# StanfordASL/RiskAverseTrajOpt

Measured on AMD Instinct MI355X. Metric: SAA constraint-eval throughput, higher is better.
Workload: dtype f32

## Files before the change

riskaversetrajopt_amd/csrc/rato_sample_launch.h:

```cpp
#pragma once
#include "rato_common.h"
#include "rato_rows_plan.h"
#include "rato_select.h"

namespace rato {

struct StatsRequest {
  void* workspace;
  double* out;
  double alpha;
  float thr;
  int flags;
  bool ok(const float* Z) const { return !workspace || (Z && out && alpha > 0.0 && alpha <= 1.0); }
};
template <class Params>
StatsRequest stats_request(const Params* p) {
  return {p->stats_workspace, p->stats_out, p->stats_alpha, p->stats_thr, p->stats_flags};
}

struct StatsPlacement {
  rato_sel::StatsTail tail;
  int grid;
  size_t lds;
  bool behind;
};
template <int NT>
int place_stats(const StatsRequest& rq, int64_t M, int grid, size_t lds, bool may_carry, StatsPlacement& sp) {
  sp = {{}, grid, lds, rq.workspace && !may_carry};
  if (!rq.workspace || !may_carry) return RATO_OK;
  const int extra = rato_sel::stats_tail_workgroups<NT>(M, sp.tail.G);
  if (extra < 0) return RATO_EINVAL;
  sp.tail.ws = static_cast<rato_sel::Workspace*>(rq.workspace);
  sp.tail.out = rq.out;
  sp.tail.alpha = rq.alpha;
  sp.tail.thr = rq.thr;
  sp.tail.n_prod = grid;
  rato_sel::stats_rank(M, rq.alpha, sp.tail.k, sp.tail.var_is_max);
  sp.grid = grid + extra;
  if (sp.lds < rato_sel::rs_body_lds_bytes<NT>()) sp.lds = rato_sel::rs_body_lds_bytes<NT>();
  return RATO_OK;
}
inline int stats_behind(const StatsRequest& rq, bool behind, const float* Z, int64_t M, void* stream) {
  if (!behind) return RATO_OK;
  return rato_risk_stats(Z, M, rq.alpha, rq.thr, rq.workspace, rato_risk_stats_workspace_bytes(M), rq.out, stream);
}

struct RowsLaunch {
  rato_rows_plan plan;
  unsigned* queue;
  StatsPlacement stats;
};
template <int NT, class PlanWith>
int prepare_rows_launch(PlanWith&& plan_with, TileQueuePool& pool, unsigned* (*resolve)(), hipStream_t st,
                        const StatsRequest& rq, int64_t M, size_t lds, RowsLaunch& rl) {
  rl.plan = plan_with(true);
  rl.queue = rl.plan.wants_queue ? pool.take(st, resolve) : nullptr;
  if (rl.plan.wants_queue && !rl.queue) rl.plan = plan_with(false);
  return place_stats<NT>(rq, M, rl.plan.workgroups, lds, !rl.queue, rl.stats);
}

}
```

riskaversetrajopt_amd/csrc/rato_select.h:

```cpp
#ifndef RATO_SELECT_H
#define RATO_SELECT_H

#include <math.h>

#include "rato_common.h"

namespace rato_sel {

constexpr unsigned long long RS_COOP_WAIT_TICKS = 10ull * 100000000ull;
constexpr int B1 = 2048, B2 = 2048, B3 = 1024;
constexpr int RS_MAX_BLOCKS = 1024;

struct Workspace {
  unsigned hist1[B1];
  unsigned hist2[B2];
  unsigned hist3[B3];
  double blockpart[RS_MAX_BLOCKS][6];
  float tstar;
  unsigned nblocks;
  unsigned magic;
  unsigned ticket;
  unsigned sig[8];
};
constexpr int SIG_Z_COUNT = 0, SIG_Z_READY = 2;
constexpr unsigned RS_MAGIC = 0x52A70517u;

__device__ __forceinline__ unsigned key_of(float f) {
  unsigned u = __float_as_uint(f);
  if (u == 0x80000000u) u = 0u;
  return (u & 0x80000000u) ? ~u : (u | 0x80000000u);
}
__device__ __forceinline__ float value_of(unsigned k) {
  const unsigned u = (k & 0x80000000u) ? (k & 0x7fffffffu) : ~k;
  return __uint_as_float(u);
}

template <int NB, int NT = RATO_BLOCK>
__device__ void find_bin(const unsigned* __restrict__ hist, unsigned k, unsigned& bin, unsigned& krem) {
  constexpr int PER = NB / NT;
  static_assert(PER >= 1 && PER * NT == NB, "bins must divide evenly over the threads");
  __shared__ unsigned wsum[NT / RATO_WAVE];
  __shared__ unsigned res[2];
  const int tid = threadIdx.x, lane = tid & 63, wave = tid >> 6;
  unsigned local[PER], tot = 0;
#pragma unroll
  for (int i = 0; i < PER; ++i) {
    local[i] = hist[tid * PER + i];
    tot += local[i];
  }
  const unsigned incl = rato::wave_scan_dpp(tot);
  if (lane == 63) wsum[wave] = incl;
  __syncthreads();
  unsigned base = 0;
  for (int w = 0; w < wave; ++w) base += wsum[w];
  unsigned excl = base + incl - tot;
  if (k >= excl && k < excl + tot) {
    unsigned run = excl;
#pragma unroll
    for (int i = 0; i < PER; ++i) {
      if (k >= run && k < run + local[i]) {
        res[0] = tid * PER + i;
        res[1] = k - run;
      }
      run += local[i];
    }
  }
  __syncthreads();
  bin = res[0];
  krem = res[1];
  __syncthreads();
}

template <int NB, int NT = RATO_BLOCK>
__device__ void flush_hist(unsigned* lds_hist, unsigned* __restrict__ ghist) {
  __syncthreads();
  for (int i = threadIdx.x; i < NB; i += NT) {
    const unsigned c = lds_hist[i];
    if (c) atomicAdd(&ghist[i], c);
  }
}


__device__ bool wait_signal(unsigned* flag) {
  __shared__ unsigned s_ok;
  if (threadIdx.x == 0) {
    const unsigned long long t_start = wall_clock64();
    unsigned ok = 1;
    for (unsigned tries = 0; __hip_atomic_load(flag, __ATOMIC_RELAXED, __HIP_MEMORY_SCOPE_AGENT) == 0u; ++tries) {
      if ((tries & 255u) == 255u && wall_clock64() - t_start > RS_COOP_WAIT_TICKS) {
        ok = 0;
        break;
      }
      __builtin_amdgcn_s_sleep(32);
    }
    __builtin_amdgcn_fence(__ATOMIC_ACQUIRE, "agent");
    s_ok = ok;
  }
  __syncthreads();
  const bool ok = s_ok != 0;
  __syncthreads();
  return ok;
}


constexpr long RS_SMALL_MAX = 12 * 1024;
constexpr int RS_COOP_KEYS = 16;
constexpr int RS_COOP_MAX_WG = 64;

template <int NB, int NT>
__device__ bool find_bin_coop(const unsigned* __restrict__ hist, unsigned k, unsigned expected, unsigned& bin,
                              unsigned& krem, unsigned& bincount) {
  constexpr int PER = NB / NT;
  static_assert(PER >= 1 && PER * NT == NB, "bins must divide evenly over the threads");
  __shared__ unsigned wsum[NT / RATO_WAVE];
  __shared__ unsigned res[3];
  const int tid = threadIdx.x, lane = tid & 63, wave = tid >> 6;
  const unsigned long long t_start = wall_clock64();
  for (unsigned tries = 0;; ++tries) {
    unsigned local[PER], tot = 0;
#pragma unroll
    for (int i = 0; i < PER; ++i) {
      local[i] = __hip_atomic_load(const_cast<unsigned*>(hist) + tid * PER + i, __ATOMIC_RELAXED, __HIP_MEMORY_SCOPE_AGENT);
      tot += local[i];
    }
    const unsigned incl = rato::wave_scan_dpp(tot);
    if (lane == 63) wsum[wave] = incl;
    __syncthreads();
    unsigned base = 0, grand = 0;
    for (int w = 0; w < NT / RATO_WAVE; ++w) {
      const unsigned v = wsum[w];
      if (w < wave) base += v;
      grand += v;
    }
    if (grand == expected) {
      const unsigned excl = base + incl - tot;
      if (k >= excl && k < excl + tot) {
        unsigned run = excl;
#pragma unroll
        for (int i = 0; i < PER; ++i) {
          if (k >= run && k < run + local[i]) {
            res[0] = tid * PER + i;
            res[1] = k - run;
            res[2] = local[i];
          }
          run += local[i];
        }
      }
      __syncthreads();
      bin = res[0];
      krem = res[1];
      bincount = res[2];
      __syncthreads();
      return true;
    }
    if (grand > expected) return false;
    if ((tries & 1023u) == 1023u) {
      if (tid == 0) res[0] = (wall_clock64() - t_start > RS_COOP_WAIT_TICKS) ? 1u : 0u;
      __syncthreads();
      const unsigned expired = res[0];
      __syncthreads();
      if (expired) return false;
    }
    __syncthreads();
    if (tries < 64) __builtin_amdgcn_s_sleep(4); else __builtin_amdgcn_s_sleep(32);
  }
}


__device__ __forceinline__ unsigned wave_min_u32_dpp(unsigned a) {
  const int top = (int)0xffffffffu;
  a = min(a, (unsigned)__builtin_amdgcn_update_dpp(top, (int)a, 0x111, 0xf, 0xf, false));
  a = min(a, (unsigned)__builtin_amdgcn_update_dpp(top, (int)a, 0x112, 0xf, 0xf, false));
  a = min(a, (unsigned)__builtin_amdgcn_update_dpp(top, (int)a, 0x114, 0xf, 0xf, false));
  a = min(a, (unsigned)__builtin_amdgcn_update_dpp(top, (int)a, 0x118, 0xf, 0xf, false));
  a = min(a, (unsigned)__builtin_amdgcn_update_dpp(top, (int)a, 0x142, 0xa, 0xf, false));
  a = min(a, (unsigned)__builtin_amdgcn_update_dpp(top, (int)a, 0x143, 0xc, 0xf, false));
  return (unsigned)__builtin_amdgcn_readlane((int)a, 63);
}
__device__ __forceinline__ unsigned wave_max_u32_dpp(unsigned a) {
  a = max(a, (unsigned)__builtin_amdgcn_update_dpp(0, (int)a, 0x111, 0xf, 0xf, false));
  a = max(a, (unsigned)__builtin_amdgcn_update_dpp(0, (int)a, 0x112, 0xf, 0xf, false));
  a = max(a, (unsigned)__builtin_amdgcn_update_dpp(0, (int)a, 0x114, 0xf, 0xf, false));
  a = max(a, (unsigned)__builtin_amdgcn_update_dpp(0, (int)a, 0x118, 0xf, 0xf, false));
  a = max(a, (unsigned)__builtin_amdgcn_update_dpp(0, (int)a, 0x142, 0xa, 0xf, false));
  a = max(a, (unsigned)__builtin_amdgcn_update_dpp(0, (int)a, 0x143, 0xc, 0xf, false));
  return (unsigned)__builtin_amdgcn_readlane((int)a, 63);
}

constexpr int RS_CAND_MAX = 256;

template <int NT>
__device__ void rs_small_body(const float* __restrict__ Z, long M, double alpha, unsigned k, int var_is_max, float thr,
                              double* __restrict__ out, unsigned* sig, unsigned* h, double* red, float* redmax,
                              unsigned* magic = nullptr) {
  constexpr int KEYS = (int)(RS_SMALL_MAX / NT), NW = NT / RATO_WAVE;
  static_assert(RS_CAND_MAX + 8 <= B1, "the candidate list reuses the histogram's LDS");
  if (sig) {
    const bool tagged = !magic || *magic == RS_MAGIC;
    const bool ok = tagged && wait_signal(sig + SIG_Z_READY);
    if (!ok) {
      if (threadIdx.x < RATO_N_STATS) out[threadIdx.x] = __longlong_as_double(0x7ff8000000000000LL);
      if (magic && threadIdx.x == 0) *magic = 0u;
      return;
    }
    if (threadIdx.x == 0) __hip_atomic_store(sig + SIG_Z_READY, 0u, __ATOMIC_RELAXED, __HIP_MEMORY_SCOPE_AGENT);
  }
  const int tid = threadIdx.x;
  const int n = (int)M;
#ifdef RATO_RS_DIAG
  if (tid == 0) out[16 + 0] = (double)wall_clock64();
#endif
  unsigned key[KEYS];
  double sum = 0.0, cnt = 0.0;
  float mx = -INFINITY;
  unsigned kmin = 0xffffffffu, kmax = 0u;
  {
    float z[KEYS];
#pragma unroll
    for (int u = 0; u < KEYS; ++u) {
      const int i = tid + u * NT;
      z[u] = (i < n) ? Z[i] : 0.0f;
    }
#pragma unroll
    for (int u = 0; u < KEYS; ++u) {
      const int i = tid + u * NT;
      key[u] = key_of(z[u]);
      if (i < n) {
        sum += (double)z[u];
        cnt += (z[u] <= thr) ? 1.0 : 0.0;
        mx = fmaxf(mx, z[u]);
        kmin = min(kmin, key[u]);
        kmax = max(kmax, key[u]);
      }
    }
  }
  unsigned* mm = reinterpret_cast<unsigned*>(red);
  kmin = wave_min_u32_dpp(kmin);
  kmax = wave_max_u32_dpp(kmax);
  if ((tid & 63) == 0) {
    mm[tid >> 6] = kmin;
    mm[NW + (tid >> 6)] = kmax;
  }
  __syncthreads();
#pragma unroll
  for (int w = 0; w < NW; ++w) {
    kmin = min(kmin, mm[w]);
    kmax = max(kmax, mm[NW + w]);
  }
#ifdef RATO_RS_DIAG
  if (tid == 0) out[16 + 1] = (double)wall_clock64();
#endif
  unsigned lo = kmin, krem = k;
  const unsigned range = kmax - kmin;
  int sh = (range == 0u) ? 0 : (32 - __clz((int)range)) - 11;
  if (sh < 0) sh = 0;
  unsigned width = 0u;
  unsigned tkey = 0u;
  for (int level = 0;; ++level) {
    for (int i = tid; i < B1; i += NT) h[i] = 0;
    __syncthreads();
    {
      unsigned run_bin = 0xffffffffu, run_cnt = 0;
#pragma unroll
      for (int u = 0; u < KEYS; ++u) {
        const int i = tid + u * NT;
        const unsigned rel = key[u] - lo;
        if (i < n && (level == 0 || (key[u] >= lo && rel < width))) {
          const unsigned bin = rel >> sh;
          if (bin != run_bin) {
            if (run_cnt) atomicAdd(&h[run_bin], run_cnt);
            run_bin = bin;
            run_cnt = 0;
// ... 19 lines not shown
      unsigned* cand = h;
      if (tid == 0) h[B1 - 2] = 0u;
      __syncthreads();
#pragma unroll
      for (int u = 0; u < KEYS; ++u) {
        const int i = tid + u * NT;
        if (i < n && key[u] >= lo && key[u] - lo < width) cand[atomicAdd(&h[B1 - 2], 1u)] = key[u];
      }
      __syncthreads();
      if (tid < (int)c) {
        const unsigned x = cand[tid];
        unsigned lt = 0, le = 0;
        for (unsigned j = 0; j < c; ++j) {
          const unsigned y = cand[j];
          lt += (y < x) ? 1u : 0u;
          le += (y <= x) ? 1u : 0u;
        }
        if (lt <= krem && krem < le) h[B1 - 1] = x;
      }
      __syncthreads();
      tkey = h[B1 - 1];
      break;
    }
    sh = (sh > 11) ? sh - 11 : 0;
  }
#ifdef RATO_RS_DIAG
  if (tid == 0) out[16 + 6] = (double)wall_clock64();
#endif
  const float t = value_of(tkey);
  double tail = 0.0, ngt = 0.0, neq = 0.0;
#pragma unroll
  for (int u = 0; u < KEYS; ++u) {
    const int i = tid + u * NT;
    if (i < n) {
      const float z = value_of(key[u]);
      tail += (key[u] > tkey) ? ((double)z - (double)t) : 0.0;
      ngt += (key[u] > tkey) ? 1.0 : 0.0;
      neq += (key[u] == tkey) ? 1.0 : 0.0;
    }
  }
#ifdef RATO_RS_DIAG
  if (tid == 0) out[16 + 7] = (double)wall_clock64();
#endif
  sum = rato::wave_sum_dpp(sum);
  cnt = rato::wave_sum_dpp(cnt);
  tail = rato::wave_sum_dpp(tail);
  ngt = rato::wave_sum_dpp(ngt);
  neq = rato::wave_sum_dpp(neq);
  mx = rato::wave_max_dpp(mx);
  __syncthreads();
  if ((tid & 63) == 0) {
    const int w = tid >> 6;
    red[0 * NW + w] = sum; red[1 * NW + w] = cnt; red[2 * NW + w] = tail; red[3 * NW + w] = ngt; red[4 * NW + w] = neq;
    redmax[w] = mx;
  }
  __syncthreads();
  if (tid < RATO_WAVE) {
    static_assert(NT / RATO_WAVE <= 16, "one DPP row folds the wave totals");
    const bool in = tid < NT / RATO_WAVE;
    const double S = rato::row16_sum_dpp(in ? red[0 * NW + tid] : 0.0), C = rato::row16_sum_dpp(in ? red[1 * NW + tid] : 0.0);
    const double T = rato::row16_sum_dpp(in ? red[2 * NW + tid] : 0.0), NG = rato::row16_sum_dpp(in ? red[3 * NW + tid] : 0.0);
    const double NE = rato::row16_sum_dpp(in ? red[4 * NW + tid] : 0.0);
    const double m = (double)rato::row16_max_dpp(in ? redmax[tid] : -INFINITY);
    if (tid == 15) {
      out[0] = var_is_max ? m : (double)t;
      out[1] = (double)t + (T / (double)M) / alpha;
      out[2] = C / (double)M;
      out[3] = S / (double)M;
      out[4] = m;
      out[5] = C;
      out[6] = T;
      out[7] = (double)k;
      out[8] = NG;
      out[9] = NE;
      out[10] = (double)t;
#ifdef RATO_RS_DIAG
      out[16 + 8] = (double)wall_clock64();
#endif
    }
  }
}


template <int NT>
__device__ void rs_coop_body(const float* __restrict__ Z, long M, double alpha, unsigned k, int var_is_max, float thr, int G,
                             Workspace* __restrict__ ws, double* __restrict__ out, int bid, int companion, unsigned* h,
                             double* red) {
  constexpr int NW = NT / RATO_WAVE;
  const int tid = threadIdx.x;
  if (ws->magic != RS_MAGIC) {
    if (bid == 0 && tid < RATO_N_STATS) out[tid] = __longlong_as_double(0x7ff8000000000000LL);
    return;
  }
  const bool z_ok = companion ? wait_signal(ws->sig + SIG_Z_READY) : true;
  __shared__ unsigned last_flag;
  const int n = (int)M;
  unsigned key[RS_COOP_KEYS];
  double sum = 0.0, cnt = 0.0;
  float mx = -INFINITY;
  {
    float z[RS_COOP_KEYS];
#pragma unroll
    for (int u = 0; u < RS_COOP_KEYS; ++u) {
      const int i = (u * G + bid) * NT + tid;
      z[u] = (i < n) ? Z[i] : 0.0f;
    }
    for (int i = tid; i < B1; i += NT) h[i] = 0;
    __syncthreads();
    unsigned run_bin = 0xffffffffu, run_cnt = 0;
#pragma unroll
    for (int u = 0; u < RS_COOP_KEYS; ++u) {
      const int i = (u * G + bid) * NT + tid;
      key[u] = key_of(z[u]);
      if (i < n) {
        const unsigned bin = key[u] >> 21;
        if (bin != run_bin) {
          if (run_cnt) atomicAdd(&h[run_bin], run_cnt);
          run_bin = bin;
          run_cnt = 0;
        }
        ++run_cnt;
        sum += (double)z[u];
        cnt += (z[u] <= thr) ? 1.0 : 0.0;
        mx = fmaxf(mx, z[u]);
      }
    }
    if (run_cnt) atomicAdd(&h[run_bin], run_cnt);
  }
  flush_hist<B1, NT>(h, ws->hist1);
  unsigned b1 = 0, k1 = 0, c1 = 0, b2 = 0, k2 = 0, c2 = 0, b3 = 0, k3 = 0, c3 = 0;
  bool ok = z_ok && find_bin_coop<B1, NT>(ws->hist1, k, (unsigned)n, b1, k1, c1);
  for (int i = tid; i < B2; i += NT) h[i] = 0;
  __syncthreads();
#pragma unroll
  for (int u = 0; u < RS_COOP_KEYS; ++u) {
    const int i = (u * G + bid) * NT + tid;
    if (i < n && (key[u] >> 21) == b1) atomicAdd(&h[(key[u] >> 10) & (B2 - 1)], 1u);
  }
  flush_hist<B2, NT>(h, ws->hist2);
  ok = ok && find_bin_coop<B2, NT>(ws->hist2, k1, c1, b2, k2, c2);
  for (int i = tid; i < B3; i += NT) h[i] = 0;
  __syncthreads();
  const unsigned prefix = (b1 << 11) | b2;
#pragma unroll
  for (int u = 0; u < RS_COOP_KEYS; ++u) {
    const int i = (u * G + bid) * NT + tid;
    if (i < n && (key[u] >> 10) == prefix) atomicAdd(&h[key[u] & (B3 - 1)], 1u);
  }
  flush_hist<B3, NT>(h, ws->hist3);
  ok = ok && find_bin_coop<B3, NT>(ws->hist3, k2, c2, b3, k3, c3);
  if (!ok) {
    if (tid < RATO_N_STATS) out[tid] = __longlong_as_double(0x7ff8000000000000LL);
    if (tid == 0) ws->magic = 0;
    return;
  }
  const unsigned tkey = (b1 << 21) | (b2 << 10) | b3;
  const float t = value_of(tkey);
  double tail = 0.0, ngt = 0.0, neq = 0.0;
#pragma unroll
  for (int u = 0; u < RS_COOP_KEYS; ++u) {
    const int i = (u * G + bid) * NT + tid;
    if (i < n) {
      const float z = value_of(key[u]);
      tail += (key[u] > tkey) ? ((double)z - (double)t) : 0.0;
      ngt += (key[u] > tkey) ? 1.0 : 0.0;
      neq += (key[u] == tkey) ? 1.0 : 0.0;
    }
  }
  sum = rato::wave_sum_dpp(sum);
  cnt = rato::wave_sum_dpp(cnt);
  tail = rato::wave_sum_dpp(tail);
  ngt = rato::wave_sum_dpp(ngt);
  neq = rato::wave_sum_dpp(neq);
  mx = rato::wave_max_dpp(mx);
  if ((tid & 63) == 0) {
    const int w = tid >> 6;
    red[0 * NW + w] = sum; red[1 * NW + w] = cnt; red[2 * NW + w] = (double)mx; red[3 * NW + w] = tail; red[4 * NW + w] = ngt; red[5 * NW + w] = neq;
  }
  __syncthreads();
  if (tid < RATO_WAVE) {
    const bool in = tid < NT / RATO_WAVE;
    const double S = rato::row16_sum_dpp(in ? red[0 * NW + tid] : 0.0), C = rato::row16_sum_dpp(in ? red[1 * NW + tid] : 0.0);
    const double T = rato::row16_sum_dpp(in ? red[3 * NW + tid] : 0.0), NG = rato::row16_sum_dpp(in ? red[4 * NW + tid] : 0.0);
    const double NE = rato::row16_sum_dpp(in ? red[5 * NW + tid] : 0.0);
    const double m = (double)rato::row16_max_dpp(in ? (float)red[2 * NW + tid] : -INFINITY);
    if (tid == 15) {
      double* bp = ws->blockpart[bid];
      bp[0] = S; bp[1] = C; bp[2] = m; bp[3] = T; bp[4] = NG; bp[5] = NE;
      const unsigned tk = __hip_atomic_fetch_add(&ws->ticket, 1u, __ATOMIC_ACQ_REL, __HIP_MEMORY_SCOPE_AGENT);
      last_flag = (tk == (unsigned)G - 1u);
    }
  }
  __syncthreads();
  if (!last_flag) return;
  for (int i = tid; i < B1 + B2 + B3; i += NT) ws->hist1[i] = 0;
  if (tid == 0) {
    ws->ticket = 0;
    if (companion) __hip_atomic_store(ws->sig + SIG_Z_READY, 0u, __ATOMIC_RELAXED, __HIP_MEMORY_SCOPE_AGENT);
  }
  if (tid >= RATO_WAVE) return;
  double s = 0, c = 0, m = -INFINITY, tl = 0, g = 0, e = 0;
  if (tid < G) {
    const double* bp = ws->blockpart[tid];
    s = __hip_atomic_load(bp + 0, __ATOMIC_RELAXED, __HIP_MEMORY_SCOPE_AGENT);
    c = __hip_atomic_load(bp + 1, __ATOMIC_RELAXED, __HIP_MEMORY_SCOPE_AGENT);
    m = __hip_atomic_load(bp + 2, __ATOMIC_RELAXED, __HIP_MEMORY_SCOPE_AGENT);
    tl = __hip_atomic_load(bp + 3, __ATOMIC_RELAXED, __HIP_MEMORY_SCOPE_AGENT);
    g = __hip_atomic_load(bp + 4, __ATOMIC_RELAXED, __HIP_MEMORY_SCOPE_AGENT);
    e = __hip_atomic_load(bp + 5, __ATOMIC_RELAXED, __HIP_MEMORY_SCOPE_AGENT);
  }
  s = rato::wave_sum_dpp(s);
  c = rato::wave_sum_dpp(c);
  tl = rato::wave_sum_dpp(tl);
  g = rato::wave_sum_dpp(g);
  e = rato::wave_sum_dpp(e);
  m = (double)rato::wave_max_dpp((float)m);
  if (tid != 0) return;
  out[0] = var_is_max ? m : (double)t;
  out[1] = (double)t + (tl / (double)M) / alpha;
  out[2] = c / (double)M;
  out[3] = s / (double)M;
  out[4] = m;
  out[5] = c;
  out[6] = tl;
  out[7] = (double)k;
  out[8] = g;
  out[9] = e;
  out[10] = (double)t;
}


struct StatsTail {
  Workspace* ws;
  double* out;
  double alpha;
  unsigned k;
  int var_is_max;
  float thr;
  int G;
  int n_prod;
  __device__ bool is_stats(int b) const { return ws && b >= n_prod; }
};

inline void stats_rank(int64_t M, double alpha, unsigned& k, int& var_is_max) {
  long xth = (long)floor(alpha * (double)M);
  long kk = (long)M - xth - 1;
  var_is_max = 0;
  if (kk < 0) {
    kk = 0;
    var_is_max = 1;
  }
  k = (unsigned)kk;
}

template <int NT>
inline int stats_tail_workgroups(int64_t M, int& G) {
  if (M <= RS_SMALL_MAX) {
    G = 0;
    return 1;
  }
  long g = (M + (long)NT * 4 - 1) / ((long)NT * 4);
  if (g > RS_COOP_MAX_WG) g = RS_COOP_MAX_WG;
  if ((long)g * NT * RS_COOP_KEYS < M) return -1;
  G = (int)g;
  return (int)g;
}

template <int NT>
__device__ __forceinline__ void stats_tail_run(const StatsTail& t, const float* __restrict__ Z, long M, unsigned char* lds) {
  unsigned* h = reinterpret_cast<unsigned*>(lds);
  double* red = reinterpret_cast<double*>(h + B1);
  float* redmax = reinterpret_cast<float*>(red + 6 * (NT / RATO_WAVE));
  if (t.G == 0) rs_small_body<NT>(Z, M, t.alpha, t.k, t.var_is_max, t.thr, t.out, t.ws->sig, h, red, redmax, &t.ws->magic);
  else rs_coop_body<NT>(Z, M, t.alpha, t.k, t.var_is_max, t.thr, t.G, t.ws, t.out, (int)blockIdx.x - t.n_prod, 1, h, red);
}

template <int NT>
constexpr size_t rs_body_lds_bytes() { return sizeof(unsigned) * B1 + sizeof(double) * 6 * (NT / RATO_WAVE) + sizeof(float) * (NT / RATO_WAVE); }


}
#endif
```

riskaversetrajopt_amd/csrc/stats.hip:

```cpp
#include <stdlib.h>

#include <atomic>

#include "rato_common.h"
#include "rato_select.h"

namespace {
using namespace rato_sel;

constexpr int SP_COLS = 16, SP_ROWS = 64;

template <typename T>
__device__ __forceinline__ void sum_partials_block(int col_block, const T* __restrict__ part, int nblocks,
                                                   int ncols, double scale, double* __restrict__ out) {
  __shared__ double red[SP_ROWS][SP_COLS + 1];
  const int cx = threadIdx.x % SP_COLS, ry = threadIdx.x / SP_COLS;
  const int c = col_block * SP_COLS + cx;
  double a0 = 0.0, a1 = 0.0, a2 = 0.0, a3 = 0.0;
  if (c < ncols) {
    int b = ry;
    for (; b + 3 * SP_ROWS < nblocks; b += 4 * SP_ROWS) {
      const T v0 = part[(size_t)b * ncols + c];
      const T v1 = part[(size_t)(b + SP_ROWS) * ncols + c];
      const T v2 = part[(size_t)(b + 2 * SP_ROWS) * ncols + c];
// ... 172 lines not shown
    if (blockIdx.x == 0) ws->tstar = t;
  }
}

__global__ __launch_bounds__(RATO_BLOCK) void rs_final(long M, double alpha, unsigned k, int var_is_max, int nblocks,
                                                        Workspace* __restrict__ ws, double* __restrict__ out) {
  const bool ok = ws->magic == RS_MAGIC;
  for (int i = threadIdx.x; i < B1 + B2 + B3; i += RATO_BLOCK) ws->hist1[i] = 0;
  if (!ok) {
    if (threadIdx.x < RATO_N_STATS) out[threadIdx.x] = __longlong_as_double(0x7ff8000000000000LL);
    return;
  }
  if (threadIdx.x >= RATO_WAVE) return;
  const int lane = threadIdx.x;
  double s = 0, c = 0, m = -INFINITY, tail = 0, ngt = 0, neq = 0;
  for (int b = lane; b < nblocks; b += RATO_WAVE) {
    s += ws->blockpart[b][0];
    c += ws->blockpart[b][1];
    m = fmax(m, ws->blockpart[b][2]);
    tail += ws->blockpart[b][3];
    ngt += ws->blockpart[b][4];
    neq += ws->blockpart[b][5];
  }
  s = rato::wave_sum(s);
  c = rato::wave_sum(c);
  tail = rato::wave_sum(tail);
  ngt = rato::wave_sum(ngt);
  neq = rato::wave_sum(neq);
#pragma unroll
  for (int off = 32; off > 0; off >>= 1) m = fmax(m, __shfl_xor(m, off, RATO_WAVE));
  if (lane != 0) return;
  const double t = (double)ws->tstar;
  out[0] = var_is_max ? m : t;
  out[1] = t + (tail / (double)M) / alpha;
  out[2] = c / (double)M;
  out[3] = s / (double)M;
  out[4] = m;
  out[5] = c;
  out[6] = tail;
  out[7] = (double)k;
  out[8] = ngt;
  out[9] = neq;
  out[10] = t;
}

constexpr int RS1_T = 1024;

__global__ __launch_bounds__(RS1_T) void rs_small(const float* __restrict__ Z, long M, double alpha, unsigned k,
                                                  int var_is_max, float thr, double* __restrict__ out,
                                                  const float* __restrict__ part, int nblocks, int ncols,
                                                  double scale, double* __restrict__ sums_out) {
  if (blockIdx.x > 0) {
    sum_partials_block(blockIdx.x - 1, part, nblocks, ncols, scale, sums_out);
    return;
  }
  __shared__ unsigned h[B1];
  __shared__ double red[5 * (RS1_T / RATO_WAVE)];
  __shared__ float redmax[RS1_T / RATO_WAVE];
  rs_small_body<RS1_T>(Z, M, alpha, k, var_is_max, thr, out, nullptr, h, red, redmax);
}

__global__ __launch_bounds__(RS1_T) void rs_small_tab(const rato::BatchProb* __restrict__ tab, long M) {
  __shared__ unsigned h[B1];
  __shared__ double red[5 * (RS1_T / RATO_WAVE)];
  __shared__ float redmax[RS1_T / RATO_WAVE];
  const rato::BatchProb& t = tab[blockIdx.x];
  rs_small_body<RS1_T>(t.m_out, M, t.alpha, t.k, t.var_is_max, t.thr, t.res_dev, nullptr, h, red, redmax);
}

__global__ __launch_bounds__(RS1_T) void rs_small_batch(const float* __restrict__ Z, long M, long ldz, double alpha, unsigned k,
                                                        int var_is_max, float thr, double* __restrict__ out) {
  __shared__ unsigned h[B1];
  __shared__ double red[5 * (RS1_T / RATO_WAVE)];
  __shared__ float redmax[RS1_T / RATO_WAVE];
  rs_small_body<RS1_T>(Z + (size_t)blockIdx.x * ldz, M, alpha, k, var_is_max, thr, out + (size_t)blockIdx.x * RATO_N_STATS, nullptr,
                       h, red, redmax);
}

constexpr long RS_COOP_MAX = (long)RS_COOP_MAX_WG * RS1_T * RS_COOP_KEYS;

__global__ __launch_bounds__(RS1_T) void rs_coop(const float* __restrict__ Z, long M, double alpha, unsigned k,
                                                 int var_is_max, float thr, int G, Workspace* __restrict__ ws,
                                                 double* __restrict__ out, const float* __restrict__ part, int nblocks,
                                                 int ncols, double scale, double* __restrict__ sums_out) {
  if ((int)blockIdx.x >= G) {
    sum_partials_block(blockIdx.x - G, part, nblocks, ncols, scale, sums_out);
    return;
  }
  __shared__ unsigned h[B1];
  __shared__ double red[6 * (RS1_T / RATO_WAVE)];
  rs_coop_body<RS1_T>(Z, M, alpha, k, var_is_max, thr, G, ws, out, (int)blockIdx.x, 0, h, red);
}

__global__ __launch_bounds__(RATO_BLOCK) void rs_init_kernel(Workspace* __restrict__ ws) {
  unsigned* w = reinterpret_cast<unsigned*>(ws);
  const int n = (int)(sizeof(Workspace) / sizeof(unsigned));
  for (int i = blockIdx.x * RATO_BLOCK + threadIdx.x; i < n; i += gridDim.x * RATO_BLOCK) w[i] = 0;
  __syncthreads();
  if (blockIdx.x == 0 && threadIdx.x == 0) ws->magic = RS_MAGIC;
}

__global__ __launch_bounds__(RATO_BLOCK) void unpack_records_kernel(const unsigned char* __restrict__ all, int world,
                                                                    int n_sums, long M_local, long rec_bytes,
                                                                    double* __restrict__ total,
                                                                    float* __restrict__ Z_all) {
  const long n = (long)world * M_local;
  for (long i = (long)blockIdx.x * RATO_BLOCK + threadIdx.x; i < n; i += (long)gridDim.x * RATO_BLOCK) {
    const long r = i / M_local, j = i - r * M_local;
    Z_all[i] = reinterpret_cast<const float*>(all + r * rec_bytes + 8L * n_sums)[j];
  }
  if (blockIdx.x == 0) {
    for (int c = threadIdx.x; c < n_sums; c += RATO_BLOCK) {
      double acc = reinterpret_cast<const double*>(all)[c];
      for (int r = 1; r < world; ++r) acc += reinterpret_cast<const double*>(all + (long)r * rec_bytes)[c];
      total[c] = acc;
    }
  }
}

}

extern "C" int rato_unpack_records(const void* all, int32_t world, int32_t n_sums, int64_t M_local, int64_t rec_bytes,
                                   double* total, float* Z_all, void* stream) {
  RATO_CLEAR_ERROR();
  if (!all || (!total && n_sums > 0) || !Z_all || world < 1 || n_sums < 0 || M_local <= 0 || rec_bytes < 8L * n_sums + 4 * M_local ||
      rec_bytes % 8 != 0)
    return RATO_EINVAL;
  long nb = ((long)world * M_local + RATO_BLOCK * 4 - 1) / (RATO_BLOCK * 4);
  if (nb > 2048) nb = 2048;
  if (nb < 1) nb = 1;
  hipLaunchKernelGGL(unpack_records_kernel, dim3((unsigned)nb), dim3(RATO_BLOCK), 0, rato::as_stream(stream),
                     static_cast<const unsigned char*>(all), world, n_sums, (long)M_local, (long)rec_bytes, total, Z_all);
  RATO_LAUNCH_CHECK();
  return RATO_OK;
}

extern "C" int rato_sum_partials(const float* part, int32_t nblocks, int32_t ncols, double scale, double* out,
                                 void* stream) {
  RATO_CLEAR_ERROR();
  if (!part || !out || nblocks <= 0 || ncols <= 0) return RATO_EINVAL;
  dim3 grid((ncols + SP_COLS - 1) / SP_COLS), block(SP_COLS * SP_ROWS);
  hipLaunchKernelGGL(sum_partials_kernel<float>, grid, block, 0, rato::as_stream(stream), part, nblocks, ncols, scale, out);
  RATO_LAUNCH_CHECK();
  return RATO_OK;
}

extern "C" int rato_sum_partials_f64(const double* part, int32_t nblocks, int32_t ncols, double scale, double* out,
                                     void* stream) {
  RATO_CLEAR_ERROR();
  if (!part || !out || nblocks <= 0 || ncols <= 0) return RATO_EINVAL;
  dim3 grid((ncols + SP_COLS - 1) / SP_COLS), block(SP_COLS * SP_ROWS);
  hipLaunchKernelGGL(sum_partials_kernel<double>, grid, block, 0, rato::as_stream(stream), part, nblocks, ncols, scale, out);
  RATO_LAUNCH_CHECK();
  return RATO_OK;
}

namespace rato {
bool risk_stats_batch_applies(int64_t M) {
  const char* e = getenv("RATO_RS_PATH");
  return M > 0 && M <= RS_SMALL_MAX && !(e && (e[0] == 'm' || e[0] == 'c'));
}

int launch_risk_stats_batch(const BatchProb* tab, int n, int64_t M, hipStream_t st) {
  RATO_CLEAR_ERROR();
  if (!tab || n < 1 || n > 65535 || !risk_stats_batch_applies(M)) return RATO_EINVAL;
  hipLaunchKernelGGL(rs_small_tab, dim3((unsigned)n), dim3(RS1_T), 0, st, tab, (long)M);
  RATO_LAUNCH_CHECK();
  return RATO_OK;
}

int launch_cut_finish_batch(const BatchProb* tab, int n, int nblocks, int ncols, int n_stats, hipStream_t st) {
  RATO_CLEAR_ERROR();
  if (!tab || n < 1 || n > 65535 || nblocks < 1 || ncols < 0) return RATO_EINVAL;
  const int col_blocks = ncols > 0 ? (ncols + SP_COLS - 1) / SP_COLS : 0;
// ... 70 lines not shown
__global__ __launch_bounds__(RATO_BLOCK) void histogram_kernel(const float* __restrict__ Z, long M, float lo, float hi,
                                                               float inv_w, int bins, unsigned* __restrict__ counts) {
  __shared__ unsigned h[HG_MAX_BINS + 3];
  const int n = bins + 3;
  for (int i = threadIdx.x; i < n; i += RATO_BLOCK) h[i] = 0;
  __syncthreads();
  int cur = 0;
  unsigned run = 0;
  for (long i = (long)blockIdx.x * RATO_BLOCK + threadIdx.x; i < M; i += (long)gridDim.x * RATO_BLOCK) {
    const int slot = histogram_slot(Z[i], lo, hi, inv_w, bins);
    if (slot != cur) {
      if (run) atomicAdd(&h[cur], run);
      cur = slot;
      run = 0;
    }
    ++run;
  }
  if (run) atomicAdd(&h[cur], run);
  __syncthreads();
  for (int i = threadIdx.x; i < n; i += RATO_BLOCK) {
    const unsigned v = h[i];
    if (v) atomicAdd(&counts[i], v);
  }
}
}

extern "C" int rato_histogram(const float* Z, int64_t M, float lo, float hi, int32_t bins, uint32_t* counts, void* stream) {
  RATO_CLEAR_ERROR();
  if (!Z || !counts || M < 1 || bins < 1 || bins > HG_MAX_BINS || !isfinite(lo) || !isfinite(hi) || !(lo < hi)) return RATO_EINVAL;
  const float width = hi - lo;
  const float inv_w = (float)bins / width;
  if (!isfinite(width) || !isfinite(inv_w)) return RATO_EINVAL;
  hipStream_t st = rato::as_stream(stream);
  hipError_t e = hipMemsetAsync(counts, 0, sizeof(uint32_t) * (size_t)(bins + 3), st);
  if (e != hipSuccess) return RATO_EHIP - (int)e;
  long nb = (M + (long)RATO_BLOCK * HG_PER_THREAD - 1) / ((long)RATO_BLOCK * HG_PER_THREAD);
  if (nb > HG_MAX_BLOCKS) nb = HG_MAX_BLOCKS;
  hipLaunchKernelGGL(histogram_kernel, dim3((unsigned)nb), dim3(RATO_BLOCK), 0, st, Z, (long)M, lo, hi, inv_w, (int)bins, counts);
  RATO_LAUNCH_CHECK();
  return RATO_OK;
}

extern "C" size_t rato_risk_stats_workspace_bytes(int64_t M) {
  (void)M;
  return sizeof(Workspace);
}

namespace {
int risk_stats_impl(const float* Z, int64_t M, double alpha, float thr, void* workspace, size_t workspace_bytes,
                    double* out, const float* part, int32_t nblocks, int32_t ncols, double scale, double* sums_out,
                    void* stream, bool recover = false) {
  RATO_CLEAR_ERROR();
  if (!Z || !out || !workspace || M <= 0 || M >= (int64_t)0xffffffffLL || !(alpha > 0.0) || !(alpha <= 1.0))
    return RATO_EINVAL;
  if (workspace_bytes < sizeof(Workspace)) return RATO_EINVAL;
  if (part && (!sums_out || nblocks <= 0 || ncols <= 0)) return RATO_EINVAL;
  long xth = (long)floor(alpha * (double)M);
  long kk = M - xth - 1;
  int var_is_max = 0;
  if (kk < 0) {
    kk = 0;
    var_is_max = 1;
  }
  const unsigned k = (unsigned)kk;
  hipStream_t st = rato::as_stream(stream);
  Workspace* ws = static_cast<Workspace*>(workspace);
  const int sp_blocks = part ? (ncols + SP_COLS - 1) / SP_COLS : 0;
  static const int force_multi_env = [] { const char* e = getenv("RATO_RS_PATH"); return (e && e[0] == 'm') ? 1 : 0; }();
  const int force_multi = force_multi_env || recover;
  static const int force_coop = [] { const char* e = getenv("RATO_RS_PATH"); return (e && e[0] == 'c') ? 1 : 0; }();
  if (M <= RS_SMALL_MAX && !force_multi && !force_coop) {
    hipLaunchKernelGGL(rs_small, dim3(1 + sp_blocks), dim3(RS1_T), 0, st, Z, (long)M, alpha, k, var_is_max, thr, out,
                       part, (int)nblocks, (int)ncols, scale, sums_out);
    RATO_LAUNCH_CHECK();
    return RATO_OK;
  }
  static const int no_coop = [] { const char* e = getenv("RATO_RS_COOP"); return (e && e[0] == '0') ? 1 : 0; }();
  if (M <= RS_COOP_MAX && !force_multi && (!no_coop || force_coop)) {
    static const int kpt_env = rato::env_int("RATO_RS_KPT", 0);
    const long kpt = (kpt_env >= 1 && kpt_env <= RS_COOP_KEYS) ? kpt_env : 4;
    long G = (M + RS1_T * kpt - 1) / (RS1_T * kpt);
    if (G > RS_COOP_MAX_WG) G = RS_COOP_MAX_WG;
    hipLaunchKernelGGL(rs_coop, dim3((unsigned)G + sp_blocks), dim3(RS1_T), 0, st, Z, (long)M, alpha, k, var_is_max, thr,
                       (int)G, ws, out, part, (int)nblocks, (int)ncols, scale, sums_out);
    RATO_LAUNCH_CHECK();
    return RATO_OK;
  }
  if (part) {
    hipLaunchKernelGGL(sum_partials_kernel<float>, dim3(sp_blocks), dim3(SP_COLS * SP_ROWS), 0, st, part, (int)nblocks,
                       (int)ncols, scale, sums_out);
  }
  long nb = (M + RATO_BLOCK * 4 - 1) / (RATO_BLOCK * 4);
  if (nb > 256) {
    nb = (M + RATO_BLOCK * 16 - 1) / (RATO_BLOCK * 16);
    if (nb < 256) nb = 256;
  }
  if (nb > RS_MAX_BLOCKS) nb = RS_MAX_BLOCKS;
  if (nb < 1) nb = 1;
  dim3 grid((unsigned)nb), block(RATO_BLOCK);
  hipLaunchKernelGGL(rs_pass1, grid, block, 0, st, Z, (long)M, thr, ws);
  hipLaunchKernelGGL(rs_pass2, grid, block, 0, st, Z, (long)M, k, ws);
  hipLaunchKernelGGL(rs_pass3, grid, block, 0, st, Z, (long)M, k, ws);
  hipLaunchKernelGGL(rs_tail, grid, block, 0, st, Z, (long)M, k, ws);
  hipLaunchKernelGGL(rs_final, dim3(1), dim3(RATO_BLOCK), 0, st, (long)M, alpha, k, var_is_max, (int)nb, ws, out);
  RATO_LAUNCH_CHECK();
  return RATO_OK;
}
}

extern "C" int rato_risk_stats_init(void* workspace, size_t workspace_bytes, void* stream) {
  RATO_CLEAR_ERROR();
  if (!workspace || workspace_bytes < sizeof(Workspace)) return RATO_EINVAL;
  hipLaunchKernelGGL(rs_init_kernel, dim3(1), dim3(RATO_BLOCK), 0, rato::as_stream(stream),
                     static_cast<Workspace*>(workspace));
  RATO_LAUNCH_CHECK();
  return RATO_OK;
}

extern "C" int rato_risk_stats(const float* Z, int64_t M, double alpha, float thr, void* workspace,
                               size_t workspace_bytes, double* out, void* stream) {
  return risk_stats_impl(Z, M, alpha, thr, workspace, workspace_bytes, out, nullptr, 0, 0, 1.0, nullptr, stream);
}

extern "C" int rato_risk_stats_batch(const float* Z, int64_t M, int64_t ldz, int32_t K, double alpha, float thr, void* workspace,
                                     size_t workspace_bytes, double* out, void* stream) {
  RATO_CLEAR_ERROR();
  if (!Z || !out || M <= 0 || ldz < M || K < 1 || !(alpha > 0.0) || !(alpha <= 1.0)) return RATO_EINVAL;
  if (M <= RS_SMALL_MAX && K <= 65535) {
    unsigned k;
    int var_is_max;
    stats_rank(M, alpha, k, var_is_max);
    hipLaunchKernelGGL(rs_small_batch, dim3((unsigned)K), dim3(RS1_T), 0, rato::as_stream(stream), Z, (long)M, (long)ldz, alpha, k,
                       var_is_max, thr, out);
    RATO_LAUNCH_CHECK();
    return RATO_OK;
  }
  for (int32_t i = 0; i < K; ++i) {
    const int rc = rato_risk_stats(Z + (size_t)i * ldz, M, alpha, thr, workspace, workspace_bytes, out + (size_t)i * RATO_N_STATS, stream);
    if (rc != RATO_OK) return rc;
  }
  return RATO_OK;
}

extern "C" int rato_risk_stats_recover(const float* Z, int64_t M, double alpha, float thr, void* workspace,
                                       size_t workspace_bytes, double* out, void* stream) {
  const int rc = rato_risk_stats_init(workspace, workspace_bytes, stream);
  if (rc != RATO_OK) return rc;
  return risk_stats_impl(Z, M, alpha, thr, workspace, workspace_bytes, out, nullptr, 0, 0, 1.0, nullptr, stream, true);
}

extern "C" int rato_sums_and_risk_stats(const float* part, int32_t nblocks, int32_t ncols, double scale,
                                        double* sums_out, const float* Z, int64_t M, double alpha, float thr,
                                        void* workspace, size_t workspace_bytes, double* out, void* stream) {
  if (!part) return RATO_EINVAL;
  return risk_stats_impl(Z, M, alpha, thr, workspace, workspace_bytes, out, part, nblocks, ncols, scale, sums_out,
                         stream);
}
```

Measured before the change: 9.568 billion.

## Guess the VaR bin window from the previous call to skip radix passes

The cooperative radix-select records the key range and threshold from each call in the workspace. On the next call it histograms keys into a narrow window centred on the previous threshold. If the target bin holds at most 256 keys, those candidates are gathered in global memory and ranked directly, which skips the second and third histogram passes and their grid-wide syncs. If too many keys land in the bin, it falls back to a full first pass plus the usual refinement and backs off exponentially before guessing again. This adds per-call state, extra min/max reductions and atomics, and a spin-wait on the candidate list.

```diff
diff --git a/riskaversetrajopt_amd/csrc/rato_sample_launch.h b/riskaversetrajopt_amd/csrc/rato_sample_launch.h
--- a/riskaversetrajopt_amd/csrc/rato_sample_launch.h
+++ b/riskaversetrajopt_amd/csrc/rato_sample_launch.h
@@ -35,6 +35,7 @@
   sp.tail.alpha = rq.alpha;
   sp.tail.thr = rq.thr;
   sp.tail.n_prod = grid;
+  sp.tail.guess = rato_sel::guess_enabled();
   rato_sel::stats_rank(M, rq.alpha, sp.tail.k, sp.tail.var_is_max);
   sp.grid = grid + extra;
   if (sp.lds < rato_sel::rs_body_lds_bytes<NT>()) sp.lds = rato_sel::rs_body_lds_bytes<NT>();
diff --git a/riskaversetrajopt_amd/csrc/rato_select.h b/riskaversetrajopt_amd/csrc/rato_select.h
--- a/riskaversetrajopt_amd/csrc/rato_select.h
+++ b/riskaversetrajopt_amd/csrc/rato_select.h
@@ -2,6 +2,7 @@
 #define RATO_SELECT_H
 
 #include <math.h>
+#include <stddef.h>
 
 #include "rato_common.h"
 
@@ -10,6 +11,7 @@
 constexpr unsigned long long RS_COOP_WAIT_TICKS = 10ull * 100000000ull;
 constexpr int B1 = 2048, B2 = 2048, B3 = 1024;
 constexpr int RS_MAX_BLOCKS = 1024;
+constexpr int RS_CAND_MAX = 256;
 
 struct Workspace {
   unsigned hist1[B1];
@@ -20,8 +22,26 @@
   unsigned nblocks;
   unsigned magic;
   unsigned ticket;
+  unsigned histx[B1];
+  unsigned long long cand[RS_CAND_MAX];
+  unsigned seq;
+  unsigned has_centre;
+  unsigned nkmin, kmax;
+  unsigned guess;
+  float g_lo, g_scale;
+  unsigned backoff, skip;
+  float g_centre;
+  unsigned n_guessed, n_fellback;
   unsigned sig[8];
 };
+static_assert(sizeof(Workspace) == offsetof(Workspace, sig) + 8 * sizeof(unsigned) &&
+              offsetof(Workspace, sig) == offsetof(Workspace, n_fellback) + sizeof(unsigned),
+              "sig ends the workspace without padding, the tallies sit right before it");
+static_assert(offsetof(Workspace, cand) % 8 == 0 && offsetof(Workspace, seq) == offsetof(Workspace, cand) + 8 * RS_CAND_MAX,
+              "the candidates are 8-byte words, stored and loaded whole");
+constexpr unsigned RS_BACKOFF_MAX = 63u;
+constexpr unsigned RS_GUESS_SET = 1u;
+constexpr float RS_WINDOW_GROWTH = 4.0f, RS_WINDOW_FIRST = 64.0f, RS_WINDOW_FINEST = 512.0f;
 constexpr int SIG_Z_COUNT = 0, SIG_Z_READY = 2;
 constexpr unsigned RS_MAGIC = 0x52A70517u;
 
@@ -186,8 +206,6 @@
   a = max(a, (unsigned)__builtin_amdgcn_update_dpp(0, (int)a, 0x143, 0xc, 0xf, false));
   return (unsigned)__builtin_amdgcn_readlane((int)a, 63);
 }
-
-constexpr int RS_CAND_MAX = 256;
 
 template <int NT>
 __device__ void rs_small_body(const float* __restrict__ Z, long M, double alpha, unsigned k, int var_is_max, float thr,
@@ -373,22 +391,99 @@
 }
 
 
+inline int guess_enabled() {
+  static const int v = rato::env_int("RATO_RS_GUESS", 1);
+  return v != 0;
+}
+
+__device__ __forceinline__ unsigned guess_bin(unsigned key, float lo, float scale) {
+#pragma clang fp contract(off)
+  const float z = value_of(key);
+  float x = (z - lo) * scale;
+  x = fminf(fmaxf(x, 0.0f), (float)(B1 - 1));
+  unsigned b = (unsigned)(int)x;
+  if (z != z) b = (key & 0x80000000u) ? (unsigned)(B1 - 1) : 0u;
+  return b;
+}
+
+template <int NB, int NT>
+__device__ void flush_hist_base(unsigned* lds_hist, unsigned* __restrict__ ghist, unsigned (&base)[NB / NT]) {
+  __syncthreads();
+#pragma unroll
+  for (int j = 0; j < NB / NT; ++j) {
+    const int i = threadIdx.x + j * NT;
+    const unsigned c = lds_hist[i];
+    base[j] = 0u;
+    if (c) base[j] = __hip_atomic_fetch_add(&ghist[i], c, __ATOMIC_RELAXED, __HIP_MEMORY_SCOPE_AGENT);
+  }
+}
+
+__device__ bool gather_candidates(unsigned long long* cand, unsigned c, unsigned stamp, unsigned krem, unsigned* keys,
+                                  unsigned* s_key, unsigned* s_ok) {
+  if (threadIdx.x < RATO_WAVE) {
+    const unsigned lane = threadIdx.x;
+    const unsigned long long t_start = wall_clock64();
+    unsigned ok = 1, x = 0u;
+    for (unsigned tries = 0;; ++tries) {
+      bool all = true;
+#pragma unroll
+      for (int j = 0; j < RS_CAND_MAX / RATO_WAVE; ++j) {
+        const unsigned i = lane + j * RATO_WAVE;
+        if (i < c) {
+          const unsigned long long e = __hip_atomic_load(cand + i, __ATOMIC_RELAXED, __HIP_MEMORY_SCOPE_AGENT);
+          if ((unsigned)(e >> 32) == stamp) {
+            keys[i] = (unsigned)e;
+            if (j == 0) x = (unsigned)e;
+          } else {
+            all = false;
+          }
+        }
+      }
+      if (__all(all)) break;
+      if ((tries & 255u) == 255u && wall_clock64() - t_start > RS_COOP_WAIT_TICKS) {
+        ok = 0;
+      }
+      if (__any(ok == 0u)) {
+        ok = 0;
+        break;
+      }
+      if (tries < 64) __builtin_amdgcn_s_sleep(2); else __builtin_amdgcn_s_sleep(32);
+    }
+    if (ok && c <= (unsigned)RATO_WAVE) {
+      unsigned lt = 0, le = 0;
+      for (unsigned j = 0; j < c; ++j) {
+        const unsigned y = (unsigned)__builtin_amdgcn_readlane((int)x, (int)j);
+        lt += (y < x) ? 1u : 0u;
+        le += (y <= x) ? 1u : 0u;
+      }
+      if (lane < c && lt <= krem && krem < le) *s_key = x;
+    }
+    if (lane == 0) *s_ok = ok;
+  }
+  __syncthreads();
+  return *s_ok != 0;
+}
+
 template <int NT>
 __device__ void rs_coop_body(const float* __restrict__ Z, long M, double alpha, unsigned k, int var_is_max, float thr, int G,
-                             Workspace* __restrict__ ws, double* __restrict__ out, int bid, int companion, unsigned* h,
-                             double* red) {
+                             Workspace* __restrict__ ws, double* __restrict__ out, int bid, int companion, int guess_on,
+                             unsigned* h, double* red) {
   constexpr int NW = NT / RATO_WAVE;
+  static_assert(RS_CAND_MAX <= NT && RS_CAND_MAX + 2 * NW + 8 <= B1, "one candidate per thread; the list and the wave extrema share the histogram's LDS");
   const int tid = threadIdx.x;
   if (ws->magic != RS_MAGIC) {
     if (bid == 0 && tid < RATO_N_STATS) out[tid] = __longlong_as_double(0x7ff8000000000000LL);
     return;
   }
+  const bool guessed = guess_on && ws->guess == RS_GUESS_SET;
+  const float g_lo = ws->g_lo, g_scale = ws->g_scale;
   const bool z_ok = companion ? wait_signal(ws->sig + SIG_Z_READY) : true;
   __shared__ unsigned last_flag;
   const int n = (int)M;
   unsigned key[RS_COOP_KEYS];
   double sum = 0.0, cnt = 0.0;
   float mx = -INFINITY;
+  unsigned kmin = 0xffffffffu, kmax = 0u;
   {
     float z[RS_COOP_KEYS];
 #pragma unroll
@@ -404,7 +499,7 @@
       const int i = (u * G + bid) * NT + tid;
       key[u] = key_of(z[u]);
       if (i < n) {
-        const unsigned bin = key[u] >> 21;
+        const unsigned bin = guessed ? guess_bin(key[u], g_lo, g_scale) : key[u] >> 21;
         if (bin != run_bin) {
           if (run_cnt) atomicAdd(&h[run_bin], run_cnt);
           run_bin = bin;
@@ -414,38 +509,106 @@
         sum += (double)z[u];
         cnt += (z[u] <= thr) ? 1.0 : 0.0;
         mx = fmaxf(mx, z[u]);
+        kmin = min(kmin, key[u]);
+        kmax = max(kmax, key[u]);
       }
     }
     if (run_cnt) atomicAdd(&h[run_bin], run_cnt);
   }
-  flush_hist<B1, NT>(h, ws->hist1);
+  unsigned slot0[B1 / NT];
+  if (guessed) flush_hist_base<B1, NT>(h, ws->hist1, slot0);
+  else flush_hist<B1, NT>(h, ws->hist1);
   unsigned b1 = 0, k1 = 0, c1 = 0, b2 = 0, k2 = 0, c2 = 0, b3 = 0, k3 = 0, c3 = 0;
   bool ok = z_ok && find_bin_coop<B1, NT>(ws->hist1, k, (unsigned)n, b1, k1, c1);
-  for (int i = tid; i < B2; i += NT) h[i] = 0;
-  __syncthreads();
-#pragma unroll
-  for (int u = 0; u < RS_COOP_KEYS; ++u) {
-    const int i = (u * G + bid) * NT + tid;
-    if (i < n && (key[u] >> 21) == b1) atomicAdd(&h[(key[u] >> 10) & (B2 - 1)], 1u);
-  }
-  flush_hist<B2, NT>(h, ws->hist2);
-  ok = ok && find_bin_coop<B2, NT>(ws->hist2, k1, c1, b2, k2, c2);
-  for (int i = tid; i < B3; i += NT) h[i] = 0;
-  __syncthreads();
-  const unsigned prefix = (b1 << 11) | b2;
-#pragma unroll
-  for (int u = 0; u < RS_COOP_KEYS; ++u) {
-    const int i = (u * G + bid) * NT + tid;
-    if (i < n && (key[u] >> 10) == prefix) atomicAdd(&h[key[u] & (B3 - 1)], 1u);
-  }
-  flush_hist<B3, NT>(h, ws->hist3);
-  ok = ok && find_bin_coop<B3, NT>(ws->hist3, k2, c2, b3, k3, c3);
+  unsigned tkey = 0u;
+  bool ranked = false;
+  const unsigned bin_guessed = b1;
+  if (guessed && ok) {
+    if (c1 <= (unsigned)RS_CAND_MAX) {
+      const unsigned stamp = ws->seq + 1u;
+      if (tid == 0) h[B1 - 2] = 0u;
+#pragma unroll
+      for (int j = 0; j < B1 / NT; ++j)
+        if ((unsigned)(tid + j * NT) == b1) h[B1 - 3] = slot0[j];
+      __syncthreads();
+      const unsigned base = h[B1 - 3];
+#pragma unroll
+      for (int u = 0; u < RS_COOP_KEYS; ++u) {
+        const int i = (u * G + bid) * NT + tid;
+        if (i < n && guess_bin(key[u], g_lo, g_scale) == b1) {
+          const unsigned s = base + atomicAdd(&h[B1 - 2], 1u);
+          if (base < (unsigned)RS_CAND_MAX && s < (unsigned)RS_CAND_MAX)
+            __hip_atomic_store(&ws->cand[s], ((unsigned long long)stamp << 32) | key[u], __ATOMIC_RELAXED, __HIP_MEMORY_SCOPE_AGENT);
+        }
+      }
+      ok = gather_candidates(ws->cand, c1, stamp, k1, h, &h[B1 - 1], &h[B1 - 4]);
+      if (ok && c1 <= (unsigned)RATO_WAVE) {
+        tkey = h[B1 - 1];
+        ranked = true;
+      } else if (ok) {
+        if ((unsigned)tid < c1) {
+          const unsigned x = h[tid];
+          unsigned lt = 0, le = 0;
+          for (unsigned j = 0; j < c1; ++j) {
+            const unsigned y = h[j];
+            lt += (y < x) ? 1u : 0u;
+            le += (y <= x) ? 1u : 0u;
+          }
+          if (lt <= k1 && k1 < le) h[B1 - 1] = x;
+        }
+        __syncthreads();
+        tkey = h[B1 - 1];
+        ranked = true;
+      }
+    } else {
+      for (int i = tid; i < B1; i += NT) h[i] = 0;
+      __syncthreads();
+      unsigned run_bin = 0xffffffffu, run_cnt = 0;
+#pragma unroll
+      for (int u = 0; u < RS_COOP_KEYS; ++u) {
+        const int i = (u * G + bid) * NT + tid;
+        if (i < n) {
+          const unsigned bin = key[u] >> 21;
+          if (bin != run_bin) {
+            if (run_cnt) atomicAdd(&h[run_bin], run_cnt);
+            run_bin = bin;
+            run_cnt = 0;
+          }
+          ++run_cnt;
+        }
+      }
+      if (run_cnt) atomicAdd(&h[run_bin], run_cnt);
+      flush_hist<B1, NT>(h, ws->histx);
+      ok = find_bin_coop<B1, NT>(ws->histx, k, (unsigned)n, b1, k1, c1);
+    }
+  }
+  if (!ranked) {
+    for (int i = tid; i < B2; i += NT) h[i] = 0;
+    __syncthreads();
+#pragma unroll
+    for (int u = 0; u < RS_COOP_KEYS; ++u) {
+      const int i = (u * G + bid) * NT + tid;
+      if (i < n && (key[u] >> 21) == b1) atomicAdd(&h[(key[u] >> 10) & (B2 - 1)], 1u);
+    }
+    flush_hist<B2, NT>(h, ws->hist2);
+    ok = ok && find_bin_coop<B2, NT>(ws->hist2, k1, c1, b2, k2, c2);
+    for (int i = tid; i < B3; i += NT) h[i] = 0;
+    __syncthreads();
+    const unsigned prefix = (b1 << 11) | b2;
+#pragma unroll
+    for (int u = 0; u < RS_COOP_KEYS; ++u) {
+      const int i = (u * G + bid) * NT + tid;
+      if (i < n && (key[u] >> 10) == prefix) atomicAdd(&h[key[u] & (B3 - 1)], 1u);
+    }
+    flush_hist<B3, NT>(h, ws->hist3);
+    ok = ok && find_bin_coop<B3, NT>(ws->hist3, k2, c2, b3, k3, c3);
+    tkey = (b1 << 21) | (b2 << 10) | b3;
+  }
   if (!ok) {
     if (tid < RATO_N_STATS) out[tid] = __longlong_as_double(0x7ff8000000000000LL);
     if (tid == 0) ws->magic = 0;
     return;
   }
-  const unsigned tkey = (b1 << 21) | (b2 << 10) | b3;
   const float t = value_of(tkey);
   double tail = 0.0, ngt = 0.0, neq = 0.0;
 #pragma unroll
@@ -464,9 +627,18 @@
   ngt = rato::wave_sum_dpp(ngt);
   neq = rato::wave_sum_dpp(neq);
   mx = rato::wave_max_dpp(mx);
+  unsigned* wext = h + (B1 - 8 - 2 * NW);
+  if (guess_on) {
+    kmin = wave_min_u32_dpp(kmin);
+    kmax = wave_max_u32_dpp(kmax);
+  }
   if ((tid & 63) == 0) {
     const int w = tid >> 6;
     red[0 * NW + w] = sum; red[1 * NW + w] = cnt; red[2 * NW + w] = (double)mx; red[3 * NW + w] = tail; red[4 * NW + w] = ngt; red[5 * NW + w] = neq;
+    if (guess_on) {
+      wext[w] = kmin;
+      wext[NW + w] = kmax;
+    }
   }
   __syncthreads();
   if (tid < RATO_WAVE) {
@@ -475,19 +647,69 @@
     const double T = rato::row16_sum_dpp(in ? red[3 * NW + tid] : 0.0), NG = rato::row16_sum_dpp(in ? red[4 * NW + tid] : 0.0);
     const double NE = rato::row16_sum_dpp(in ? red[5 * NW + tid] : 0.0);
     const double m = (double)rato::row16_max_dpp(in ? (float)red[2 * NW + tid] : -INFINITY);
+    unsigned gmin = 0xffffffffu, gmax = 0u;
+    if (guess_on) {
+      gmin = wave_min_u32_dpp(in ? wext[tid] : 0xffffffffu);
+      gmax = wave_max_u32_dpp(in ? wext[NW + tid] : 0u);
+    }
     if (tid == 15) {
       double* bp = ws->blockpart[bid];
       bp[0] = S; bp[1] = C; bp[2] = m; bp[3] = T; bp[4] = NG; bp[5] = NE;
+      if (guess_on) {
+        __hip_atomic_fetch_max(&ws->nkmin, ~gmin, __ATOMIC_RELAXED, __HIP_MEMORY_SCOPE_AGENT);
+        __hip_atomic_fetch_max(&ws->kmax, gmax, __ATOMIC_RELAXED, __HIP_MEMORY_SCOPE_AGENT);
+      }
       const unsigned tk = __hip_atomic_fetch_add(&ws->ticket, 1u, __ATOMIC_ACQ_REL, __HIP_MEMORY_SCOPE_AGENT);
       last_flag = (tk == (unsigned)G - 1u);
     }
   }
   __syncthreads();
   if (!last_flag) return;
-  for (int i = tid; i < B1 + B2 + B3; i += NT) ws->hist1[i] = 0;
+  if (!guessed) {
+    for (int i = tid; i < B1 + B2 + B3; i += NT) ws->hist1[i] = 0;
+  } else if (ranked) {
+    for (int i = tid; i < B1; i += NT) ws->hist1[i] = 0;
+  } else {
+    for (int i = tid; i < B1 + B2 + B3; i += NT) ws->hist1[i] = 0;
+    for (int i = tid; i < B1; i += NT) ws->histx[i] = 0;
+  }
   if (tid == 0) {
     ws->ticket = 0;
     if (companion) __hip_atomic_store(ws->sig + SIG_Z_READY, 0u, __ATOMIC_RELAXED, __HIP_MEMORY_SCOPE_AGENT);
+    if (guess_on) {
+      const float zlo = value_of(~__hip_atomic_load(&ws->nkmin, __ATOMIC_RELAXED, __HIP_MEMORY_SCOPE_AGENT));
+      const float zhi = value_of(__hip_atomic_load(&ws->kmax, __ATOMIC_RELAXED, __HIP_MEMORY_SCOPE_AGENT));
+      const float range = zhi - zlo;
+      float w = ws->has_centre ? RS_WINDOW_GROWTH * fabsf(t - ws->g_centre) : range / RS_WINDOW_FIRST;
+      w = fminf(fmaxf(w, range / RS_WINDOW_FINEST), range);
+      const float lo = t - w;
+      const float scale = (float)(B1 / 2) / w;
+      const bool good = range > 0.0f && isfinite(range) && w > 0.0f && isfinite(lo) && isfinite(scale) && scale > 0.0f;
+      unsigned backoff = ws->backoff, skip = ws->skip;
+      if (guessed) {
+        ws->n_guessed += 1u;
+        if (ranked) {
+          backoff = 0u;
+        } else {
+          ws->n_fellback += 1u;
+          if (bin_guessed != 0u && bin_guessed != (unsigned)(B1 - 1)) {
+            backoff = min(2u * backoff + 1u, RS_BACKOFF_MAX);
+            skip = backoff + 1u;
+          }
+        }
+      }
+      if (skip) --skip;
+      ws->backoff = backoff;
+      ws->skip = skip;
+      ws->g_centre = t;
+      ws->has_centre = (t == t) ? 1u : 0u;
+      ws->g_lo = lo;
+      ws->g_scale = scale;
+      ws->guess = (good && skip == 0u) ? RS_GUESS_SET : 0u;
+      ws->nkmin = 0u;
+      ws->kmax = 0u;
+      ws->seq = (ws->seq + 2u == 0u) ? 0u : ws->seq + 1u;
+    }
   }
   if (tid >= RATO_WAVE) return;
   double s = 0, c = 0, m = -INFINITY, tl = 0, g = 0, e = 0;
@@ -530,6 +752,7 @@
   float thr;
   int G;
   int n_prod;
+  int guess;
   __device__ bool is_stats(int b) const { return ws && b >= n_prod; }
 };
 
@@ -563,7 +786,7 @@
   double* red = reinterpret_cast<double*>(h + B1);
   float* redmax = reinterpret_cast<float*>(red + 6 * (NT / RATO_WAVE));
   if (t.G == 0) rs_small_body<NT>(Z, M, t.alpha, t.k, t.var_is_max, t.thr, t.out, t.ws->sig, h, red, redmax, &t.ws->magic);
-  else rs_coop_body<NT>(Z, M, t.alpha, t.k, t.var_is_max, t.thr, t.G, t.ws, t.out, (int)blockIdx.x - t.n_prod, 1, h, red);
+  else rs_coop_body<NT>(Z, M, t.alpha, t.k, t.var_is_max, t.thr, t.G, t.ws, t.out, (int)blockIdx.x - t.n_prod, 1, t.guess, h, red);
 }
 
 template <int NT>
diff --git a/riskaversetrajopt_amd/csrc/stats.hip b/riskaversetrajopt_amd/csrc/stats.hip
--- a/riskaversetrajopt_amd/csrc/stats.hip
+++ b/riskaversetrajopt_amd/csrc/stats.hip
@@ -278,14 +278,14 @@
 __global__ __launch_bounds__(RS1_T) void rs_coop(const float* __restrict__ Z, long M, double alpha, unsigned k,
                                                  int var_is_max, float thr, int G, Workspace* __restrict__ ws,
                                                  double* __restrict__ out, const float* __restrict__ part, int nblocks,
-                                                 int ncols, double scale, double* __restrict__ sums_out) {
+                                                 int ncols, double scale, double* __restrict__ sums_out, int guess_on) {
   if ((int)blockIdx.x >= G) {
     sum_partials_block(blockIdx.x - G, part, nblocks, ncols, scale, sums_out);
     return;
   }
   __shared__ unsigned h[B1];
   __shared__ double red[6 * (RS1_T / RATO_WAVE)];
-  rs_coop_body<RS1_T>(Z, M, alpha, k, var_is_max, thr, G, ws, out, (int)blockIdx.x, 0, h, red);
+  rs_coop_body<RS1_T>(Z, M, alpha, k, var_is_max, thr, G, ws, out, (int)blockIdx.x, 0, guess_on, h, red);
 }
 
 __global__ __launch_bounds__(RATO_BLOCK) void rs_init_kernel(Workspace* __restrict__ ws) {
@@ -522,7 +522,7 @@
     long G = (M + RS1_T * kpt - 1) / (RS1_T * kpt);
     if (G > RS_COOP_MAX_WG) G = RS_COOP_MAX_WG;
     hipLaunchKernelGGL(rs_coop, dim3((unsigned)G + sp_blocks), dim3(RS1_T), 0, st, Z, (long)M, alpha, k, var_is_max, thr,
-                       (int)G, ws, out, part, (int)nblocks, (int)ncols, scale, sums_out);
+                       (int)G, ws, out, part, (int)nblocks, (int)ncols, scale, sums_out, rato_sel::guess_enabled());
     RATO_LAUNCH_CHECK();
     return RATO_OK;
   }
```

Result: no change. 9.619 billion, median of 6 (+0.5%).
